# zfountas/deep-active-inference-mc

Hardware: AMD Instinct MI355X
Metric: EFE rollouts/sec (64x64 dSprites, 10 MC-samples, depth 5) (higher is better)
Workload: dtype f32; 1 GPU; calculate_G_repeated: 128 rows (32 roots x 4 actions) x depth 5 x 10 MC samples per GPU (BASELINE configs[1]) + action posterior; rows_per_gpu=128, samples=10, depth=5, parallelism=episodes sharded x1, weights replicated

## Files before the change

deep-active-inference-mc_amd/csrc/decoder.hip:

```cpp
#include <utility>
#include "mfma_pipe.h"

namespace efe {

template <class F, int... I> __device__ __forceinline__ void static_for_(F&& f, std::integer_sequence<int, I...>) { (f(std::integral_constant<int, I>{}), ...); }
template <int N, class F> __device__ __forceinline__ void static_for(F&& f) { static_for_(f, std::make_integer_sequence<int, N>{}); }

__host__ __device__ constexpr int w3_nch(int G) { return G == 4 ? 5 : 4; }
__host__ __device__ constexpr int w3_prod(int G, int c) {
    return G < 4 ? 5 * ((G >> 1) + 2 * (c >> 1)) + (G & 1) + 2 * (c & 1)
         : G == 4 ? (c < 2 ? 5 * (1 + 2 * c) + 4 : c < 4 ? 20 + 1 + 2 * (c - 2) : 24)
                  : (c < 2 ? 5 * (2 * c) + 4 : 20 + 2 * (c - 2));
}
__host__ __device__ constexpr bool w3_direct(int pp) { return f22_o1(pp / 5) < 0 && f22_o1(pp % 5) < 0; }
__host__ __device__ constexpr int w3_view(int pp) { return 3 * f22_view(pp / 5) + f22_view(pp % 5); }
__host__ __device__ constexpr int w3_mat(int pp) { return 4 * f22_wt(pp / 5) + f22_wt(pp % 5); }
__host__ __device__ constexpr bool w3_hits(int pp, int o) {
    const int r = o >> 2, c = o & 3, pr = pp / 5, pc = pp % 5;
    return (r == f22_o0(pr) || r == f22_o1(pr)) && (c == f22_o0(pc) || c == f22_o1(pc));
}
__host__ __device__ constexpr bool w3_seen(int G, int c, int o) {
    for (int g = 0; g < G; ++g)
        for (int k = 0; k < w3_nch(g); ++k) if (w3_hits(w3_prod(g, k), o)) return true;
    if (!w3_direct(w3_prod(G, c)))
// ... 396 lines not shown
                for (int ct = 0; ct < 4; ++ct) {
                    const f32x4 bias4 = smv[DA_BIAS + 16 + 4 * ct + g];
                    f22_l2<FUSED>(acc2, aq, wrsrc(W2 + ct * 256), ct < 3 ? 1 : 0, ln, bias4, smv, nb);
                    if (ct < 3) f22_l2_store(acc2, yr, yoff, ct, true);
                }
                if constexpr (!FUSED) load_next(NPE, 2 * NPH);
                f22_l2_store(acc2, yr, yoff, 3, true);
                if constexpr (FUSED) tail(img, nimg, pf);
            } else {
                load_next(0, 2 * NPH);
            }
        }
        __syncthreads();
        img = nimg; nimg = FUSED ? vpark(nnimg) : nnimg;
    }
}

__global__ void __launch_bounds__(256, 2) k_dec_a(const DecAArgs a) {
    extern __shared__ __attribute__((aligned(16))) float4 sm[];
    dec_a_loop<false>(a, sm, [](int, int, f32x4 (&)[16]) {});
}

constexpr int DAS_IN = 6 * 16;
constexpr int DAS_L1 = 4 * 16;
constexpr int DAS_BIAS = (DAS_IN + 1 + DAS_L1 + 2) * DA_PS;
constexpr size_t DAS_LDS_BYTES = (DAS_BIAS + 32) * sizeof(float4);
__global__ void __launch_bounds__(256, 2) k_dec_a_s(const DecAArgs a) {
    extern __shared__ __attribute__((aligned(16))) float4 sm[];
    float4* sin = sm;
    float4* sl1 = sm + (DAS_IN + 1) * DA_PS;
// ... 68 lines not shown
constexpr size_t DA_LDS_BYTES = (DA_BIAS + 33) * sizeof(float4);
int init_dec_b_kernels();
int init_decoder_kernels() {
    if (hipFuncSetAttribute((const void*)k_dec_a, hipFuncAttributeMaxDynamicSharedMemorySize, DA_LDS_BYTES) != hipSuccess) return 1;
    if (hipFuncSetAttribute((const void*)k_dec_a_s, hipFuncAttributeMaxDynamicSharedMemorySize, DAS_LDS_BYTES) != hipSuccess) return 1;
    return init_dec_b_kernels();
}

void launch_dec_a(const DecAArgs& a, hipStream_t st) {
    if (a.parts == 8) {
        hipLaunchKernelGGL(k_dec_a_s, dim3(a.rows * 8), dim3(256), DAS_LDS_BYTES, st, a);
        return;
    }
    const size_t lds = DA_LDS_BYTES;
    const int grid = a.rows < 512 ? a.rows : 512;
    hipLaunchKernelGGL(k_dec_a, dim3(grid), dim3(256), lds, st, a);
}


template <int PARTS, bool FUSED>
__device__ __forceinline__ void dec_b_image(const DecBArgs& a, float4* const sm, float4* const sb3, float* const sq, float* const sQ,
                                            const int img, const int qtr, const float* const y2img) {
    constexpr int SR = 4, NW = 4, NTHR = 256;
    constexpr int DB_RP = 33;
    constexpr int DB_PS = 17;
    constexpr int DB_IN_F4 = (SR + 1) * DB_RP * DB_PS;
    constexpr int DB_YROWS = 4 * SR + 2;
    constexpr int NPF = (SR + 1) * 512 / NTHR;
    constexpr int NS = 32 / SR;
    float* sH = reinterpret_cast<float*>(sm + DB_IN_F4);
    int tid = threadIdx.x;
// ... 223 lines not shown
        const DecAArgs an = karg_reload<DecAArgs>(kp_lo, kp_hi, 0);
        int tl = threadIdx.x; asm volatile("" : "+v"(tl));
        const int pimg = __builtin_amdgcn_readfirstlane(nimg < an.rows ? nimg : img);
        dec_a_load_x4(pf, an.x4, pimg, __builtin_amdgcn_readfirstlane(tl >> 6), tl, 0, 16);
    }, kp_lo, kp_hi);
}

int init_dec_b_kernels() {
    if (hipFuncSetAttribute((const void*)k_dec_b4<1>, hipFuncAttributeMaxDynamicSharedMemorySize, DB_LDS4D) != hipSuccess) return 1;
    if (hipFuncSetAttribute((const void*)k_dec_b4<4>, hipFuncAttributeMaxDynamicSharedMemorySize, DB_LDS4D) != hipSuccess) return 1;
    return 0;
}

int dec_ab_grid(int rows, int cap) { const int g = rows < 512 ? rows : 512; return cap > 0 && cap < g ? cap : g; }
void launch_dec_ab(const DecABArgs& a, int grid_cap, hipStream_t st) {
    hipLaunchKernelGGL(k_dec_ab, dim3(dec_ab_grid(a.a.rows, grid_cap)), dim3(256), 0, st, a);
}

void launch_dec_b(const DecBArgs& a, hipStream_t st) {
    if (a.parts == 4) hipLaunchKernelGGL(k_dec_b4<4>, dim3(a.rows * 4), dim3(256), DB_LDS4D, st, a);
    else hipLaunchKernelGGL(k_dec_b4<1>, dim3(a.rows), dim3(256), DB_LDS4D, st, a);
}

__host__ __device__ inline int fc4_spg(int mtiles) { return ((mtiles + 7) / 8 + 7) / 8; }
template <int NT>
__global__ void __launch_bounds__(256, 2) k_fc4(const GemmArgs a) {
    constexpr int RT = 32 * NT;
    extern __shared__ __attribute__((aligned(16))) float4 sm[];
    const int tid = threadIdx.x;
    const int lane = tid & 63;
    const int w = __builtin_amdgcn_readfirstlane(tid >> 6);
// ... 93 lines not shown
```

deep-active-inference-mc_amd/csrc/engine.h:

```cpp
#pragma once
#include <hip/hip_runtime.h>
#include <algorithm>
#include <cmath>
#include <cstdio>
#include <cstring>
#include <map>
#include <mutex>
#include <string>
#include <vector>
#include "../../include/efe_engine.h"
#include "ctx_registry.h"
#include "kernels.h"

using namespace efe;

#define HIPCHK(x) do { hipError_t e_ = (x); if (e_ != hipSuccess) { return ctx->fail(std::string(#x) + ": " + hipGetErrorString(e_)); } } while (0)

namespace efe {
namespace host {

constexpr int S_DIM = 10;
constexpr int64_t MAC_TRANS = 541696, MAC_DEC = 43256320, MAC_ENC = 3868960, MAC_HABIT = 18176;
constexpr size_t SCRATCH_HEADROOM = (size_t)1 << 20;

// ... 40 lines not shown
    int pi_dim = 4, chan = 1, res = 64;
    bool generic = false;
    bool last_s1 = false;
    int base = 16, enc_hw[5] = {64, 31, 15, 7, 3};
    size_t img_store = 4096;
    Layer g_fc4, g_ct[3], g_enc[4];
    float* g_wf = nullptr; float g_bf[4] = {0.f, 0.f, 0.f, 0.f};
    float* g_enc1p = nullptr;
    int64_t mac_dec = 43256320, mac_enc = 3868960, mac_trans = 541696, mac_habit = 18176;
    MlpW dec16{}, enc16{};
    int enc16_kc0 = 0;
    int64_t head_unfused = 0;
    MlpW mid16{}, top16{};
    TrainPart top_train, mid_train;
    int64_t mid_unfused = 0;
    float *enc_w1 = nullptr, *enc_b1 = nullptr, *dec_wf = nullptr;
    float dec_bf = 0.f;
    float* dec_raw = nullptr;
    float* dect_raw = nullptr;
    float* dect_raw_g = nullptr;
    float* dec_raw_g = nullptr;
    float* enc_raw = nullptr;
    float* enc_raw_g = nullptr;
    float* down_master = nullptr;
    RepackDesc* down_repack = nullptr; int down_repack_n = 0, down_repack_blocks = 0;
    bool down_dirty = false, dec_bf_stale = false;
    float* down_master_g = nullptr;
    RepackDesc* down_repack_g = nullptr; int down_repack_g_n = 0, down_repack_g_blocks = 0;
    bool g_bf_stale = false;
    float* zeros = nullptr;
// ... 15 lines not shown
    int64_t dec_split = 1;
    int64_t dec_fuse_ab = 1;
    int64_t dec_ab_grid = 0;
    int64_t fuse_final_g = 1;
    int64_t mfma_bf16x3 = 0;
    int split_packed = 0;
    uint16_t* fc4_b3 = nullptr;
    uint16_t* ct_b3[2] = {nullptr, nullptr};
    uint16_t* ct3_b3 = nullptr;
    float s_fc4 = 1.f, s_ct[2] = {1.f, 1.f}, s_ct3 = 1.f;
    int64_t b3_convt3 = 1;
    bool arch_gfx950 = false;
    int64_t sim_split = 1;
    bool sim_sync_dirty = false;
    double* mi_ws = nullptr;
    float* sim_xch = nullptr; int* sim_sync = nullptr;
    int64_t check_rows = 0;
    int64_t last_macs = 0;
    unsigned prof = 0;
    int cls = PROF_OTHER;
    std::vector<hipEvent_t> ev_pool;
    size_t ev_used = 0;
    std::vector<std::pair<int, std::pair<hipEvent_t, hipEvent_t>>> ev_spans;
    hipEvent_t ev_get() {
        if (ev_used == ev_pool.size()) { hipEvent_t e; (void)hipEventCreate(&e); ev_pool.push_back(e); }
        return ev_pool[ev_used++];
    }
    int trace_n = 0;
    hipEvent_t prof_begin(hipStream_t st) {
        if (trace) { (void)hipStreamSynchronize(st); fprintf(stderr, "[efe trace] launch %d class %d ...\n", ++trace_n, cls); fflush(stderr); return (hipEvent_t)1; }
// ... 89 lines not shown
    hipStream_t st;
    bool ok = false, record = false;
    Call(efe_ctx* c, Mode mode, hipStream_t stream = nullptr)
        : adm(registry().admit(c)), ctx(adm.ctx.get()), dev(ctx ? ctx->device : -1), st(stream) { tl_stale_msg.clear(); ok = ctx && !start(mode); }
    int refused(const char* who) const {
        if (!ctx) tl_stale_msg = std::string(who) + ": stale or invalid context handle";
        return 1;
    }
    int start(Mode mode) {
        if (mode == Mode::scratch && !ctx->committed) return ctx->fail("weights not committed");
        if (mode != Mode::host && hipSetDevice(ctx->device) != hipSuccess) return ctx->fail("hipSetDevice failed");
        if (mode == Mode::host || mode == Mode::device) return 0;
        if (ctx->have_last && ctx->last_stream != st && !capturing(st) && hipStreamWaitEvent(st, ctx->done_ev, 0) != hipSuccess)
            return ctx->fail("hipStreamWaitEvent failed");
        ctx->arena.reset();
        if (ctx->poison >= 0)
            for (auto& b : ctx->arena.blocks)
                if (hipMemsetAsync(b.first, (int)(ctx->poison & 0xff), b.second, st) != hipSuccess) return ctx->fail("poison memset failed");
        ctx->last_macs = 0;
        record = true;
        return 0;
    }
    ~Call() {
        if (record && !capturing(st) && hipEventRecord(ctx->done_ev, st) == hipSuccess) { ctx->last_stream = st; ctx->have_last = true; }
        if (ctx) ctx->pending.clear();
    }
    explicit operator bool() const { return ok; }
    int finish() {
        if (!ctx->pending.empty()) return ctx->fail(ctx->pending);
        hipError_t e = hipGetLastError();
        return e == hipSuccess ? 0 : ctx->fail(std::string("kernel launch: ") + hipGetErrorString(e));
    }
};

LayerSpec top_layer(int i, int A);
LayerSpec mid_layer(int i, int A);
int part_param_count(int nl, LayerSpec (*layer)(int, int), int A);
int refresh_down_host(efe_ctx* ctx);
int64_t down_g_count(const efe_ctx* ctx);
int pack_fc4_b3(efe_ctx* ctx, int mode);

NoiseCfg make_noise(uint32_t k0, uint32_t k1, int rows_per_group, uint32_t row_offset, GroupMap gm, const int32_t* ids = nullptr, int div = 1,
                    const uint8_t* mask = nullptr);
NoiseCfg pass_noise(const efe_noise* nz, uint32_t pass, uint32_t sample, int M);
RolloutPlan rollout_plan(const efe_ctx* ctx, int64_t M);
size_t plan_bytes(const efe_ctx* c, const RolloutPlan& p);
DecTailPlan dec_tail_plan(int64_t M, bool own_y1, bool own_y2, bool own_y3, bool own_po);
DecHeadPlan dec_head_plan(int64_t M, bool own_h1, bool own_h2, bool own_h3, bool own_h4);
size_t encoder_bytes(const efe_ctx* ctx, int64_t N);
size_t core_bytes(const efe_ctx* ctx, int64_t R, int64_t D, int64_t S, bool own_terms);
int run_mid(efe_ctx* ctx, const float* X, int x_mod, int M, float* tr , const NoiseCfg& nc, hipStream_t st);
int run_decoder(efe_ctx* ctx, const float* dec_in , int N, const NoiseCfg& nc, int reward0, int store0,
                float* val , float* po_store, hipStream_t st);
int run_encoder(efe_ctx* ctx, const float* o, int N, const NoiseCfg& nc, float* enc, hipStream_t st);
int run_habit(efe_ctx* ctx, const float* s16 , int M, float* l32 , hipStream_t st);
int run_core(efe_ctx* ctx, const CoreIO& io, hipStream_t st);

int fe_params(efe_ctx* ctx, const efe_fe_params* p, bool derived_ok, const char* who);
void fe_omega(FeArgs& a, const efe_fe_params* p);
FeArgs fe_down_args(efe_ctx* ctx, int M, const float* o1, const float* enc, const float* p1_mean, const float* p1_lv, int p1_ld,
                    const efe_fe_params* p, const float* omega, const efe_fe_out* out);

}
}
```

deep-active-inference-mc_amd/csrc/engine_ctx.hip:

```cpp
#include "engine.h"

namespace {

void release_ctx(efe_ctx* ctx) {
    for (hipEvent_t e : ctx->ev_pool) (void)hipEventDestroy(e);
    if (ctx->done_ev) (void)hipEventDestroy(ctx->done_ev);
    for (void* p : ctx->owned) (void)hipFree(p);
    for (void* p : ctx->wbufs) (void)hipFree(p);
    for (auto& b : ctx->arena.blocks) (void)hipFree(b.first);
    delete ctx;
}
void destroy_ctx(efe_ctx* ctx) {
    DeviceScope dev_scope_(ctx->device);
    (void)hipSetDevice(ctx->device);
    (void)hipDeviceSynchronize();
    release_ctx(ctx);
}

}

namespace efe {
namespace host {

bool capturing(hipStream_t st) {
// ... 48 lines not shown
    }
    ctx->mac_trans = (int64_t)(pi_dim + 10) * 512 + 2 * 512 * 512 + 512 * 20;
    ctx->mac_habit = 10 * 128 + 128 * 128 + 128 * pi_dim;
    const size_t zeros_bytes = std::max<size_t>(8192, ((size_t)ctx->enc_hw[4] * ctx->enc_hw[4] * 64 + 64) * sizeof(float));
    if (hipMalloc((void**)&ctx->zeros, zeros_bytes) != hipSuccess) { release_ctx(ctx); return 4; }
    ctx->owned.push_back(ctx->zeros);
    if (hipMemset(ctx->zeros, 0, zeros_bytes) != hipSuccess) { release_ctx(ctx); return 4; }
    if (hipEventCreateWithFlags(&ctx->done_ev, hipEventDisableTiming) != hipSuccess) { ctx->done_ev = nullptr; release_ctx(ctx); return 6; }
    {
        const size_t xb = (size_t)SIM_MAX_SPLIT_GROUPS * 2 * 16 * 512 * sizeof(float), sb = (size_t)SIM_MAX_SPLIT_GROUPS * 4 * sizeof(int);
        if (hipMalloc((void**)&ctx->sim_xch, xb) != hipSuccess) { release_ctx(ctx); return 4; }
        ctx->owned.push_back(ctx->sim_xch);
        if (hipMalloc((void**)&ctx->sim_sync, sb) != hipSuccess) { release_ctx(ctx); return 4; }
        ctx->owned.push_back(ctx->sim_sync);
        if (hipMemset(ctx->sim_sync, 0, sb) != hipSuccess) { release_ctx(ctx); return 4; }
    }
    {
        if (hipMalloc((void**)&ctx->mi_ws, (EVAL_MI_WS + EVAL_MI_PSI) * sizeof(double)) != hipSuccess) { release_ctx(ctx); return 4; }
        ctx->owned.push_back(ctx->mi_ws);
        std::vector<double> psi(EVAL_MI_PSI);
        eval_mi_psi_table(psi.data());
        if (hipMemcpy(ctx->mi_ws + EVAL_MI_WS, psi.data(), psi.size() * sizeof(double), hipMemcpyHostToDevice) != hipSuccess) { release_ctx(ctx); return 4; }
    }
    registry().insert(ctx);
    *out = ctx;
    return 0;
}

void efe_destroy(efe_ctx* ctx) { registry().retire(ctx); }

// ... 45 lines not shown
    if (!strcmp(name, "mfma_bf16x3") || !strcmp(name, "mfma_f16x2")) {
        const int mode = !value ? 0 : name[5] == 'b' ? 1 : 2;
        if (mode && ctx->generic) return ctx->fail(std::string(name) + ": the experiment covers the Dynamic-dSprites geometry only");
        if (mode && ctx->committed && ctx->split_packed != mode) {
            HIPCHK(hipSetDevice(ctx->device));
            HIPCHK(hipDeviceSynchronize());
            if (refresh_down_host(ctx)) return 1;
            if (pack_fc4_b3(ctx, mode)) { ctx->mfma_bf16x3 = 0; return 1; }
        }
        ctx->mfma_bf16x3 = mode;
        return 0;
    }
    if (!strcmp(name, "b3_convt3")) { ctx->b3_convt3 = value ? 1 : 0; return 0; }
    if (!strcmp(name, "arena_align")) { if (value < 256 || (value & (value - 1))) return ctx->fail("arena_align must be a power of two >= 256"); ctx->arena_align = value; return 0; }
    if (!strcmp(name, "mid_unfused")) { ctx->mid_unfused = value; return 0; }
    if (!strcmp(name, "head_unfused")) { ctx->head_unfused = value; return 0; }
    if (!strcmp(name, "enc_chunk")) { if (value < 1) return ctx->fail("enc_chunk < 1"); ctx->enc_chunk = value; return 0; }
    return ctx->fail(std::string("unknown option ") + name);
}

int64_t efe_last_call_macs(efe_ctx* ctx) { Call call(ctx, Mode::host); return call ? ctx->last_macs : 0; }

int efe_prof_enable(efe_ctx* ctx, int on) {
    Call call(ctx, Mode::host); if (!call) return 1;
    ctx->prof = (on < 0) ? 0xFFFFFFFFu : (unsigned)on;
    ctx->ev_used = 0;
    ctx->ev_spans.clear();
    return 0;
}

// ... 49 lines not shown
```

deep-active-inference-mc_amd/csrc/engine_forward.hip:

```cpp
#include "engine.h"

namespace efe {
namespace host {
namespace {

inline RowMask live_of(const NoiseCfg& nc, int m0) { return RowMask{nc.mask, nc.mask_div, m0, nc.rows_per_group, nc.mask ? nc.gm.ids : nullptr}; }
template <class Args>
void set_keys(Args& a, const NoiseCfg& nc, int m0) {
    a.k0 = nc.k0; a.k1 = nc.k1; a.gm = nc.gm; a.rows_per_group = nc.rows_per_group; a.row_offset = nc.row_offset; a.m0 = m0;
}

void fc(efe_ctx* ctx, int cls, const Layer& L, const float* X, int ldx, int x_mod, float* Y, int ldy, int M, bool relu, bool drop,
        uint32_t tag, const NoiseCfg& nc, int m0, hipStream_t st, bool split16 = true) {
    GemmArgs a{};
    a.Wp = L.Wp; a.bias = L.bias; a.X = X; a.Y = Y; a.zeros = ctx->zeros;
    a.n_pix = M; a.cin = L.cin; a.cout = L.cout; a.mtiles = L.mtiles; a.ldx = ldx; a.ldy = ldy; a.x_mod = x_mod;
    a.relu = relu; a.dropout = drop; a.tag = tag;
    set_keys(a, nc, m0);
    ProfSpan span(ctx, cls, st);
    if (L.mtiles >= 64 && !(L.mtiles & 1) && L.cin == 256 && ldx == 256 && x_mod == 0 && relu && drop) {
        if (split16 && ctx->mfma_bf16x3 && ctx->fc4_b3 && &L == &ctx->dec_fc[3]) {
            a.Wb3 = ctx->fc4_b3; a.split = (int)ctx->mfma_bf16x3; a.wb3_scale_inv = 1.0f / ctx->s_fc4;
            launch_fc4_b3(a, st);
        }
// ... 241 lines not shown
    return {(int)C, G, own_y1 ? C * DEC_TAIL_Y1 : 0, own_y2 ? C * DEC_TAIL_Y2 : 0, own_y3 ? C * DEC_TAIL_Y3 : 0, own_po ? C * 4096 : 0,
            C * 4096, C * DEC_TAIL_Y3, C * DEC_TAIL_Y2, C * DEC_TAIL_Y1, G > 1 ? (size_t)G * DEC_TAIL_P : 0};
}
DecHeadPlan dec_head_plan(int64_t M, bool own_h1, bool own_h2, bool own_h3, bool own_h4) {
    const size_t C = (size_t)std::min<int64_t>(DEC_TAIL_ROWS, M);
    const int G = dec_head_slabs((int)std::min<int64_t>(M, 16 * DEC_HEAD_SLABS));
    return {(int)C, G, own_h1 ? C * 256 : 0, own_h2 ? C * 256 : 0, own_h3 ? C * 256 : 0, own_h4 ? C * DEC_TAIL_Y1 : 0, C * DEC_TAIL_Y1,
            (size_t)DEC_HEAD_SEGS * C * 256, G > 1 ? (size_t)G * DEC_HEAD_SMALL_P : 0};
}
size_t encoder_bytes(const efe_ctx* ctx, int64_t N) { return ctx->generic ? plan_bytes(ctx, enc_g_plan(ctx, N)) : plan_bytes(ctx, enc_plan(ctx, N)); }
size_t core_bytes(const efe_ctx* ctx, int64_t R, int64_t D, int64_t S, bool own_terms) {
    return plan_bytes(ctx, core_plan(ctx, R, D, S, true, own_terms)) + (size_t)D * plan_bytes(ctx, mid_plan(ctx, 2 * S * R))
         + decoder_bytes(ctx, D * 3 * S * R) + encoder_bytes(ctx, D * S * R);
}

int run_mid(efe_ctx* ctx, const float* X, int x_mod, int M, float* tr , const NoiseCfg& nc, hipStream_t st) {
    ctx->last_macs += (int64_t)M * ctx->mac_trans;
    if (!ctx->mid_unfused) {
        TransFusedArgs a{};
        a.W = ctx->mid16; a.X = X; a.tr = tr; a.M = M; a.x_mod = x_mod;
        set_keys(a, nc, 0);
        ProfSpan span(ctx, PROF_MID, st);
        launch_trans_fused(a, st);
        return 0;
    }
    const MidPlan p = mid_plan(ctx, M);
    float* h1 = ctx->allocT<float>(p.h1);
    float* h2 = ctx->allocT<float>(p.h2);
    if (!h1 || !h2) return 1;
    fc(ctx, PROF_MID, ctx->mid[0], X, 16, x_mod, h1, 512, M, true, true, TAG_MID + 0, nc, 0, st);
    fc(ctx, PROF_MID, ctx->mid[1], h1, 512, 0, h2, 512, M, true, true, TAG_MID + 1, nc, 0, st);
    fc(ctx, PROF_MID, ctx->mid[2], h2, 512, 0, h1, 512, M, true, true, TAG_MID + 2, nc, 0, st);
    fc(ctx, PROF_MID, ctx->mid[3], h1, 512, 0, tr, 32, M, false, false, 0, nc, 0, st);
    return 0;
}

// ... 10 lines not shown
    }
    const DecPlan p = dec_plan(ctx, N);
    const bool split = p.split;
    const bool f16 = ctx->mfma_bf16x3 == 2;
    const bool fc4_16 = !(f16 && split), ct3_16 = ctx->b3_convt3 || f16;
    const int C = p.C;
    float* hA = ctx->allocT<float>(p.hA);
    float* hB = ctx->allocT<float>(p.hB);
    float* x4 = ctx->allocT<float>(p.x4);
    float* y2 = ctx->allocT<float>(p.y2);
    if (!hA || !hB || !x4 || !y2) return 1;
    ctx->last_macs += (int64_t)N * ctx->mac_dec;
    dense_head(ctx, false, dec_in, 16, hA, 256, hA, hB, N, nc, 0, st);
    int* queues = ctx->allocT<int>(p.queues);
    if (!queues) return 1;
    if (!split && hipMemsetAsync(queues, 0, p.queues * sizeof(int), st) != hipSuccess) return ctx->fail("hipMemsetAsync failed");
    for (int m0 = 0; m0 < N; m0 += C) {
        const int c = std::min(C, N - m0);
        fc(ctx, PROF_DEC_FC4, ctx->dec_fc[3], hA + (size_t)m0 * 256, 256, 0, x4, 16384, c, true, true, TAG_DEC + 3, nc, m0, st, fc4_16);
        if (p.fused) {
            DecABArgs ab{};
            DecAArgs& da = ab.a; DecBArgs& db = ab.b;
            da.x4 = x4; da.y2 = y2; da.w1 = ctx->dec_ct[0].Wp; da.b1 = ctx->dec_ct[0].bias; da.w2 = ctx->dec_ct[1].Wp;
            da.b2 = ctx->dec_ct[1].bias; da.rows = c; da.live = live_of(nc, m0); da.queue = queues + m0 / C; da.parts = 1;
            db.y2 = y2; db.w3 = ctx->dec_ct[2].Wp; db.b3 = ctx->dec_ct[2].bias; db.w4 = ctx->dec_wf; db.b4 = ctx->dec_bf;
            db.rows = c; db.live = da.live; db.m0 = m0; db.rows_per_group = nc.rows_per_group; db.gm = nc.gm; db.reward0 = reward0; db.store0 = store0;
            db.val = val; db.parts = 1; db.valq = nullptr; db.po = po_store; db.reward_intent = (int)ctx->reward_intent;
            ProfSpan span(ctx, PROF_CT2, st);
            launch_dec_ab(ab, (int)ctx->dec_ab_grid, st);
            continue;
        }
        DecAArgs da{};
        da.x4 = x4; da.y2 = y2; da.w1 = ctx->dec_ct[0].Wp; da.b1 = ctx->dec_ct[0].bias; da.w2 = ctx->dec_ct[1].Wp;
        da.b2 = ctx->dec_ct[1].bias; da.rows = c; da.live = live_of(nc, m0); da.queue = queues + m0 / C; da.parts = split ? 8 : 1;
        {
            ProfSpan span(ctx, PROF_CT2, st);
            if (ctx->mfma_bf16x3 && ctx->ct_b3[0] && !split) {
                da.w1b3 = ctx->ct_b3[0]; da.w2b3 = ctx->ct_b3[1]; da.split = (int)ctx->mfma_bf16x3;
                da.w1s = ctx->s_ct[0]; da.w1s_inv = 1.0f / ctx->s_ct[0]; da.w2s = ctx->s_ct[1]; da.w2s_inv = 1.0f / ctx->s_ct[1];
                launch_dec_a_b3(da, st);
            }
            else launch_dec_a(da, st);
        }
        DecBArgs db{};
        db.y2 = y2; db.w3 = ctx->dec_ct[2].Wp; db.b3 = ctx->dec_ct[2].bias; db.w4 = ctx->dec_wf; db.b4 = ctx->dec_bf;
        db.rows = c; db.live = live_of(nc, m0); db.m0 = m0; db.rows_per_group = nc.rows_per_group; db.gm = nc.gm; db.reward0 = reward0; db.store0 = store0;
        db.val = val; db.parts = split ? 4 : 1; db.valq = split ? val : nullptr; db.po = po_store; db.reward_intent = (int)ctx->reward_intent;
        ProfSpan span(ctx, PROF_CT3, st);
        if (ctx->mfma_bf16x3 && ct3_16 && ctx->ct3_b3 && !split) {
// ... 49 lines not shown
    float* xbuf = ctx->allocT<float>(plan.xbuf);
    float* val = ctx->allocT<float>(plan.val);
    float* po_store = ctx->allocT<float>(plan.po_store);
    float* enc = ctx->allocT<float>(plan.enc);
    float* terms_tmp = io.terms ? nullptr : ctx->allocT<float>(plan.terms_tmp);
    if (!tr_all || !dec_in || !xbuf || !val || !po_store || !enc) return 1;
    auto noise = [&](const GroupMap& gm, const uint8_t* mask) { return make_noise(io.k0, io.k1, R, io.row_offset, gm, io.ids, io.mask_div, mask); };

    const float* x = io.x0;
    for (int t = 0; t < D; ++t) {
        float* tr = tr_all + (size_t)t * 2 * S * R * 32;
        if (io.pre_tr) {
        } else if (io.given_mean) {
            launch_fill_tr(io.given_mean, io.given_logvar, tr, R, st);
            if (run_mid(ctx, x, R, R, tr + (size_t)R * 32, noise(GroupMap{1, 1, {PASS_T2, 0, 0}, io.stage0 + (uint32_t)t, 0}, nullptr), st)) return 1;
        } else {
            if (run_mid(ctx, x, R, 2 * S * R, tr, noise(GroupMap{2 * S, S, {PASS_T1, PASS_T2, 0}, io.stage0 + (uint32_t)t, 0}, nullptr), st)) return 1;
        }
        TransPostArgs p{};
        p.tr = tr; p.x = x; p.eps_inj = io.eps ? io.eps + (size_t)t * 3 * S * R * 10 : nullptr;
        p.given_ps1 = io.given_ps1;
        p.dec_in = dec_in + (size_t)t * 3 * S * R * 16;
        float* nx = xbuf + (size_t)(t & 1) * R * 16;
        p.next_x = (t + 1 < D) ? nx : nullptr;
        p.ps1_last = (t + 1 == D) ? io.ps1 : nullptr;
        p.ps1_mean_last = (t + 1 == D) ? io.ps1_mean : nullptr;
        p.S = S; p.R = R; p.mean_mode = io.mean_mode; p.carry_mean = io.carry_mean;
        p.k0 = io.k0; p.k1 = io.k1; p.stage = io.stage0 + t; p.row_offset = io.row_offset; p.pi_dim = ctx->pi_dim;
        p.ids = io.ids; p.ids_div = io.mask_div;
        launch_trans_post(p, st);
        x = nx;
    }
    if (run_decoder(ctx, dec_in, D * 3 * S * R, noise(GroupMap{3 * S, S, {PASS_D1, PASS_D2A, PASS_D2B}, io.stage0, 0}, io.mask), 1, 1, val, po_store, st)) return 1;
    if (run_encoder(ctx, po_store, D * S * R, noise(GroupMap{S, S, {PASS_E1, 0, 0}, io.stage0, 0}, io.mask), enc, st)) return 1;
    TermsArgs ta{};
    ta.val = val; ta.valq = plan.vsplit ? val : nullptr; ta.tr = tr_all; ta.enc = enc; ta.D = D; ta.S = S; ta.R = R;
    ta.reward_div = ctx->generic ? 0.0f : (ctx->reward_intent ? 192.0f : 4096.0f);
    ta.G = io.G; ta.terms = io.terms ? io.terms : terms_tmp; ta.t2parts = io.t2parts;
    launch_terms(ta, st);
    if (io.po1) {
        const float* last = po_store + ((size_t)(D - 1) * S + (S - 1)) * R * ctx->img_store;
        if (ctx->generic) launch_to_nchw(last, io.po1, R, ctx->res * ctx->res, ctx->chan, st);
        else if (hipMemcpyAsync(io.po1, last, (size_t)R * 4096 * 4, hipMemcpyDeviceToDevice, st) != hipSuccess) return ctx->fail("po1 copy failed");
    }
    return 0;
// ... 5 lines not shown
```

deep-active-inference-mc_amd/csrc/fused.hip:

```cpp
#include "kernels.h"

namespace efe {

typedef float f32x4 __attribute__((ext_vector_type(4)));
typedef unsigned u32x4 __attribute__((ext_vector_type(4)));

namespace {

constexpr int FR = 16;
constexpr int ACT_F4 = FR * 128;

__device__ __forceinline__ int aswz(int n, int c4) { return n * 128 + ((c4 & ~15) | ((c4 ^ n) & 15)); }

__device__ __forceinline__ float4 wfrag16(__amdgpu_buffer_rsrc_t r, unsigned lane_bytes, unsigned f4_index) {
    const u32x4 v = __builtin_amdgcn_raw_buffer_load_b128(r, lane_bytes, f4_index * 16u, 0);
    return __builtin_bit_cast(float4, v);
}
__device__ __forceinline__ __amdgpu_buffer_rsrc_t rsrc16(const void* base) {
    return __builtin_amdgcn_make_buffer_rsrc(const_cast<void*>(base), 0, 0x7fffffff, 0x00020000);
}

#define MFMA16(ACC, AV, BV)                                                     \
    ACC = __builtin_amdgcn_mfma_f32_16x16x4f32((AV).x, (BV).x, ACC, 0, 0, 0);   \
    ACC = __builtin_amdgcn_mfma_f32_16x16x4f32((AV).y, (BV).y, ACC, 0, 0, 0);   \
// ... 154 lines not shown
        const float4 v = hidden16_slice<true, true>(W.w[1], W.b[1], mt0, 32, bufB, n, q, ln, k0, k1, TAG_MID + 1, rk);
        float* xb = xch + (size_t)(xn & 1) * (16 * 512);
        __builtin_amdgcn_raw_buffer_store_b128(__builtin_bit_cast(u32x4, v), rsrc16(xb), (unsigned)((n * XCH_ROW_F4 + 4 * mt0 + q) * 16), 0, AUX_SC1);
        xchg_gather<NWG>(xb, sync, NWG * (xn + 1), bufA, tid, bad);
        ++xn;
    }
    {
        const float4 v = hidden16_slice<true, true>(W.w[2], W.b[2], mt0, 32, bufA, n, q, ln, k0, k1, TAG_MID + 2, rk);
        float* xb = xch + (size_t)(xn & 1) * (16 * 512);
        __builtin_amdgcn_raw_buffer_store_b128(__builtin_bit_cast(u32x4, v), rsrc16(xb), (unsigned)((n * XCH_ROW_F4 + 4 * mt0 + q) * 16), 0, AUX_SC1);
        xchg_gather<NWG>(xb, sync, NWG * (xn + 1), bufB, tid, bad);
        ++xn;
    }
    if (w < 2) bufA[aswz(n, 4 * w + q)] = hidden16_slice<false, false>(W.w[3], W.b[3], w, 32, bufB, n, q, ln, k0, k1, 0u, rk);
    __syncthreads();
}

}

__global__ void __launch_bounds__(256, 2) k_trans_fused(const TransFusedArgs a) {
    extern __shared__ __attribute__((aligned(16))) float4 sm[];
    float4* bufA = sm;
    float4* bufB = sm + ACT_F4;
    const int tid = threadIdx.x, lane = tid & 63;
    const int w = __builtin_amdgcn_readfirstlane(tid >> 6);
    const int n = lane & 15, q = lane >> 4;
    const unsigned ln = (unsigned)lane * 16u;
    const int row0 = blockIdx.x * FR;
    {
        if (tid < 64) {
// ... 12 lines not shown
        const int mg = a.m0 + m;
        const int g = mg / a.rows_per_group;
        rk.row = global_row(a.gm.ids, a.gm.ids_div, mg - g * a.rows_per_group, a.row_offset);
        const uint2 key = group_key(a.gm, g);
        rk.stream = key.x; rk.stage = key.y;
    }
    __syncthreads();
    trans_chain(a.W, bufA, bufB, w, n, q, ln, a.k0, a.k1, rk);
    if (tid < 64) {
        const int m = row0 + n;
        if (m < a.M) {
            reinterpret_cast<float4*>(a.tr + (size_t)m * 32)[q] = bufA[aswz(n, q)];
            reinterpret_cast<float4*>(a.tr + (size_t)m * 32)[4 + q] = bufA[aswz(n, 4 + q)];
        }
    }
}

void launch_trans_fused(const TransFusedArgs& a, hipStream_t st) {
    hipLaunchKernelGGL(k_trans_fused, dim3((a.M + FR - 1) / FR), dim3(256), 2 * ACT_F4 * sizeof(float4), st, a);
}

template <int NWG>
__global__ void __launch_bounds__(256, 1) k_sim_chain(const SimChainArgs a) {
    extern __shared__ __attribute__((aligned(16))) float4 sm[];
    float4* bufA = sm;
    float4* bufB = sm + ACT_F4;
    float* srow = reinterpret_cast<float*>(sm + 2 * ACT_F4);
    float* sact = srow + SIM_FE * 16;
    const int A = a.pi_dim;
    const int tid = threadIdx.x, lane = tid & 63;
// ... 266 lines not shown
```

deep-active-inference-mc_amd/csrc/kernels.h:

```cpp
#pragma once
#include <hip/hip_runtime.h>
#include <stdint.h>
#include "philox.h"

namespace efe {

struct GroupMap {
    int per_stage, S;
    uint32_t pass[3];
    uint32_t stage0, sample0;
    const int32_t* ids = nullptr; int ids_div = 1;
};
__device__ __forceinline__ uint32_t global_row(const int32_t* ids, int ids_div, int r, uint32_t row_offset) {
    if (!ids) return row_offset + (uint32_t)r;
    const int e = r / ids_div;
    return row_offset + (uint32_t)(ids[e] * ids_div + (r - e * ids_div));
}
__host__ __device__ inline void group_decode(const GroupMap& gm, int g, int& t, int& pidx, int& samp) {
    t = g / gm.per_stage;
    const int q = g - t * gm.per_stage;
    pidx = q / gm.S;
    samp = q - pidx * gm.S;
}
__device__ __forceinline__ uint2 group_key(const GroupMap& gm, int g) {
// ... 50 lines not shown
    uint32_t row_offset;
    int m0;
    const void* Wb3 = nullptr;
    int split = 0;
    float wb3_scale_inv = 1.0f;
};

struct DecAArgs {
    const float* x4; float* y2;
    const float* w1; const float* b1;
    const float* w2; const float* b2;
    int rows;
    RowMask live;
    int parts;
    int* queue;
    const void* w1b3 = nullptr; const void* w2b3 = nullptr;
    int split = 0;
    float w1s = 1.0f, w1s_inv = 1.0f, w2s = 1.0f, w2s_inv = 1.0f;
};
__host__ __device__ constexpr int f22_view(int p) { return p == 4 ? 2 : (p & 1); }
__host__ __device__ constexpr int f22_wt(int p) { return p < 2 ? 0 : p - 1; }
__host__ __device__ constexpr int f22_o0(int p) { return p < 2 ? 0 : (p < 4 ? 1 : 3); }
__host__ __device__ constexpr int f22_o1(int p) { return p == 1 ? 2 : (p == 3 ? 3 : -1); }
__host__ __device__ constexpr int f22_cw(int wt, int k) { return wt == 0 ? (k == 1) : wt == 1 ? (k == 2) : wt == 2 ? (k != 1) : (k == 0); }
__host__ __device__ inline float f22_u_elem(const float* k, int wr, int wc) {
#pragma clang fp contract(off)
    double s = 0;
    for (int kh = 0; kh < 3; ++kh)
        for (int kw = 0; kw < 3; ++kw) s += (double)(f22_cw(wr, kh) * f22_cw(wc, kw)) * (double)k[kh * 3 + kw];
    return (float)s;
}
__host__ __device__ constexpr double wino_g(int a, int u) { return a == 0 ? (u == 0 ? 1.0 : 0.0) : a == 1 ? 0.5 : a == 2 ? (u == 1 ? -0.5 : 0.5) : (u == 2 ? 1.0 : 0.0); }
__host__ __device__ inline float wino_u_elem(const float* k, int a, int b) {
#pragma clang fp contract(off)
    double Gg[3];
    for (int v = 0; v < 3; ++v) {
        double s = 0;
        for (int u = 0; u < 3; ++u) s += wino_g(a, u) * (double)k[(2 - u) * 3 + (2 - v)];
        Gg[v] = s;
    }
    double s = 0;
    for (int v = 0; v < 3; ++v) s += Gg[v] * wino_g(b, v);
    return (float)s;
}

struct DecBArgs {
    const float* y2;
    const float* w3; const float* b3;
    const float* w4; float b4;
    int rows;
    RowMask live;
    int m0;
    int rows_per_group;
    GroupMap gm;
    int reward0;
    int store0;
    float* val;
    int parts;
    float* valq;
    float* po;
// ... 93 lines not shown

struct MlpW { const float4* w[4]; const float* b[4]; };
struct HeadArgs {
    MlpW W;
    int kc0;
    int nl;
    int out_tiles;
    uint32_t tag0;
    const float* X; float* Y;
    int M;
    uint32_t k0, k1;
    GroupMap gm; int rows_per_group; uint32_t row_offset; int m0;
};
void launch_head(const HeadArgs& a, hipStream_t st);

struct TransFusedArgs {
    MlpW W;
    const float* X;
    float* tr;
    int M, x_mod;
    uint32_t k0, k1;
    GroupMap gm; int rows_per_group; uint32_t row_offset; int m0;
};
void launch_trans_fused(const TransFusedArgs& a, hipStream_t st);
struct SimChainArgs {
    MlpW W, H;
    const float* s0;
    int E, T, use_means;
    uint32_t k0, k1, stage, row_offset;
    const float* eps_inj;
    const float* u_inj;
    float *s0_traj, *ps1_traj, *mean_traj, *lv_traj;
    float* pi0;
    float* Qpi0;
    float* tr;
    int pi_dim;
    const int32_t* ids;
// ... 500 lines not shown
```

Before: 12700 rollouts/s.

## Fold trans-post into fused transition kernel and self-reset decoder work queue

Adds a fold path that performs the trans_post sampling (reparameterized noise, dec_in/next_x writes) inside the fused transition MLP kernel, removing a separate launch per depth step. It also gives the decoder a persistent queue counter that the last ticket-holding block resets to zero, so the per-call hipMemsetAsync can be skipped. fold_trans_post defaults to off while fold_launches defaults to on, so only the queue self-reset is active by default. The risk is queue state desync if a launch aborts, plus duplicated noise logic in the fold path.

```diff
diff --git a/deep-active-inference-mc_amd/csrc/decoder.hip b/deep-active-inference-mc_amd/csrc/decoder.hip
--- a/deep-active-inference-mc_amd/csrc/decoder.hip
+++ b/deep-active-inference-mc_amd/csrc/decoder.hip
@@ -434,6 +434,12 @@
         __syncthreads();
         img = nimg; nimg = FUSED ? vpark(nnimg) : nnimg;
     }
+    int te_ = tid; asm volatile("" : "+v"(te_));
+    if (te_ == 0) {
+        int* const queue = FUSED ? karg_reload<int*>(kp_lo, kp_hi, __builtin_offsetof(DecAArgs, queue)) : a_.queue;
+        const int last = FUSED ? karg_reload<int>(kp_lo, kp_hi, __builtin_offsetof(DecAArgs, last_ticket)) : a_.last_ticket;
+        if (slot[0] == last) *queue = 0;
+    }
 }
 
 __global__ void __launch_bounds__(256, 2) k_dec_a(const DecAArgs a) {
@@ -532,7 +538,9 @@
     }
     const size_t lds = DA_LDS_BYTES;
     const int grid = a.rows < 512 ? a.rows : 512;
-    hipLaunchKernelGGL(k_dec_a, dim3(grid), dim3(256), lds, st, a);
+    DecAArgs al = a;
+    al.last_ticket = dec_last_ticket(grid, a.rows);
+    hipLaunchKernelGGL(k_dec_a, dim3(grid), dim3(256), lds, st, al);
 }
 
 
@@ -786,7 +794,10 @@
 
 int dec_ab_grid(int rows, int cap) { const int g = rows < 512 ? rows : 512; return cap > 0 && cap < g ? cap : g; }
 void launch_dec_ab(const DecABArgs& a, int grid_cap, hipStream_t st) {
-    hipLaunchKernelGGL(k_dec_ab, dim3(dec_ab_grid(a.a.rows, grid_cap)), dim3(256), 0, st, a);
+    const int grid = dec_ab_grid(a.a.rows, grid_cap);
+    DecABArgs al = a;
+    al.a.last_ticket = dec_last_ticket(grid, a.a.rows);
+    hipLaunchKernelGGL(k_dec_ab, dim3(grid), dim3(256), 0, st, al);
 }
 
 void launch_dec_b(const DecBArgs& a, hipStream_t st) {
diff --git a/deep-active-inference-mc_amd/csrc/engine.h b/deep-active-inference-mc_amd/csrc/engine.h
--- a/deep-active-inference-mc_amd/csrc/engine.h
+++ b/deep-active-inference-mc_amd/csrc/engine.h
@@ -78,6 +78,8 @@
     MlpW mid16{}, top16{};
     TrainPart top_train, mid_train;
     int64_t mid_unfused = 0;
+    int64_t fold_launches = 1;
+    int64_t fold_trans_post = 0;
     float *enc_w1 = nullptr, *enc_b1 = nullptr, *dec_wf = nullptr;
     float dec_bf = 0.f;
     float* dec_raw = nullptr;
@@ -123,6 +125,7 @@
     int64_t sim_split = 1;
     bool sim_sync_dirty = false;
     double* mi_ws = nullptr;
+    int* dec_queue = nullptr; int dec_queue_state = 0;
     float* sim_xch = nullptr; int* sim_sync = nullptr;
     int64_t check_rows = 0;
     int64_t last_macs = 0;
@@ -242,6 +245,7 @@
         if (ctx->have_last && ctx->last_stream != st && !capturing(st) && hipStreamWaitEvent(st, ctx->done_ev, 0) != hipSuccess)
             return ctx->fail("hipStreamWaitEvent failed");
         ctx->arena.reset();
+        if (ctx->dec_queue_state == 2) ctx->dec_queue_state = 1;
         if (ctx->poison >= 0)
             for (auto& b : ctx->arena.blocks)
                 if (hipMemsetAsync(b.first, (int)(ctx->poison & 0xff), b.second, st) != hipSuccess) return ctx->fail("poison memset failed");
@@ -257,6 +261,7 @@
     int finish() {
         if (!ctx->pending.empty()) return ctx->fail(ctx->pending);
         hipError_t e = hipGetLastError();
+        if (e == hipSuccess && ctx->dec_queue_state == 2) ctx->dec_queue_state = 0;
         return e == hipSuccess ? 0 : ctx->fail(std::string("kernel launch: ") + hipGetErrorString(e));
     }
 };
@@ -277,7 +282,7 @@
 DecHeadPlan dec_head_plan(int64_t M, bool own_h1, bool own_h2, bool own_h3, bool own_h4);
 size_t encoder_bytes(const efe_ctx* ctx, int64_t N);
 size_t core_bytes(const efe_ctx* ctx, int64_t R, int64_t D, int64_t S, bool own_terms);
-int run_mid(efe_ctx* ctx, const float* X, int x_mod, int M, float* tr , const NoiseCfg& nc, hipStream_t st);
+int run_mid(efe_ctx* ctx, const float* X, int x_mod, int M, float* tr , const NoiseCfg& nc, hipStream_t st, const TransFoldArgs* fold = nullptr);
 int run_decoder(efe_ctx* ctx, const float* dec_in , int N, const NoiseCfg& nc, int reward0, int store0,
                 float* val , float* po_store, hipStream_t st);
 int run_encoder(efe_ctx* ctx, const float* o, int N, const NoiseCfg& nc, float* enc, hipStream_t st);
diff --git a/deep-active-inference-mc_amd/csrc/engine_ctx.hip b/deep-active-inference-mc_amd/csrc/engine_ctx.hip
--- a/deep-active-inference-mc_amd/csrc/engine_ctx.hip
+++ b/deep-active-inference-mc_amd/csrc/engine_ctx.hip
@@ -86,6 +86,11 @@
         if (hipMalloc((void**)&ctx->sim_sync, sb) != hipSuccess) { release_ctx(ctx); return 4; }
         ctx->owned.push_back(ctx->sim_sync);
         if (hipMemset(ctx->sim_sync, 0, sb) != hipSuccess) { release_ctx(ctx); return 4; }
+    }
+    {
+        if (hipMalloc((void**)&ctx->dec_queue, 256) != hipSuccess) { release_ctx(ctx); return 4; }
+        ctx->owned.push_back(ctx->dec_queue);
+        if (hipMemset(ctx->dec_queue, 0, 256) != hipSuccess) { release_ctx(ctx); return 4; }
     }
     {
         if (hipMalloc((void**)&ctx->mi_ws, (EVAL_MI_WS + EVAL_MI_PSI) * sizeof(double)) != hipSuccess) { release_ctx(ctx); return 4; }
@@ -161,6 +166,8 @@
     if (!strcmp(name, "b3_convt3")) { ctx->b3_convt3 = value ? 1 : 0; return 0; }
     if (!strcmp(name, "arena_align")) { if (value < 256 || (value & (value - 1))) return ctx->fail("arena_align must be a power of two >= 256"); ctx->arena_align = value; return 0; }
     if (!strcmp(name, "mid_unfused")) { ctx->mid_unfused = value; return 0; }
+    if (!strcmp(name, "fold_launches")) { ctx->fold_launches = value ? 1 : 0; return 0; }
+    if (!strcmp(name, "fold_trans_post")) { ctx->fold_trans_post = value ? 1 : 0; return 0; }
     if (!strcmp(name, "head_unfused")) { ctx->head_unfused = value; return 0; }
     if (!strcmp(name, "enc_chunk")) { if (value < 1) return ctx->fail("enc_chunk < 1"); ctx->enc_chunk = value; return 0; }
     return ctx->fail(std::string("unknown option ") + name);
diff --git a/deep-active-inference-mc_amd/csrc/engine_forward.hip b/deep-active-inference-mc_amd/csrc/engine_forward.hip
--- a/deep-active-inference-mc_amd/csrc/engine_forward.hip
+++ b/deep-active-inference-mc_amd/csrc/engine_forward.hip
@@ -279,12 +279,13 @@
          + decoder_bytes(ctx, D * 3 * S * R) + encoder_bytes(ctx, D * S * R);
 }
 
-int run_mid(efe_ctx* ctx, const float* X, int x_mod, int M, float* tr , const NoiseCfg& nc, hipStream_t st) {
+int run_mid(efe_ctx* ctx, const float* X, int x_mod, int M, float* tr , const NoiseCfg& nc, hipStream_t st, const TransFoldArgs* fold) {
     ctx->last_macs += (int64_t)M * ctx->mac_trans;
     if (!ctx->mid_unfused) {
         TransFusedArgs a{};
         a.W = ctx->mid16; a.X = X; a.tr = tr; a.M = M; a.x_mod = x_mod;
         set_keys(a, nc, 0);
+        if (fold) a.fold = *fold;
         ProfSpan span(ctx, PROF_MID, st);
         launch_trans_fused(a, st);
         return 0;
@@ -325,7 +326,11 @@
     dense_head(ctx, false, dec_in, 16, hA, 256, hA, hB, N, nc, 0, st);
     int* queues = ctx->allocT<int>(p.queues);
     if (!queues) return 1;
-    if (!split && hipMemsetAsync(queues, 0, p.queues * sizeof(int), st) != hipSuccess) return ctx->fail("hipMemsetAsync failed");
+    const bool own_queue = ctx->fold_launches && !split;
+    if (own_queue) {
+        if (ctx->dec_queue_state == 1 && hipMemsetAsync(ctx->dec_queue, 0, sizeof(int), st) != hipSuccess) return ctx->fail("hipMemsetAsync failed");
+        ctx->dec_queue_state = 2;
+    } else if (!split && hipMemsetAsync(queues, 0, p.queues * sizeof(int), st) != hipSuccess) return ctx->fail("hipMemsetAsync failed");
     for (int m0 = 0; m0 < N; m0 += C) {
         const int c = std::min(C, N - m0);
         fc(ctx, PROF_DEC_FC4, ctx->dec_fc[3], hA + (size_t)m0 * 256, 256, 0, x4, 16384, c, true, true, TAG_DEC + 3, nc, m0, st, fc4_16);
@@ -333,7 +338,7 @@
             DecABArgs ab{};
             DecAArgs& da = ab.a; DecBArgs& db = ab.b;
             da.x4 = x4; da.y2 = y2; da.w1 = ctx->dec_ct[0].Wp; da.b1 = ctx->dec_ct[0].bias; da.w2 = ctx->dec_ct[1].Wp;
-            da.b2 = ctx->dec_ct[1].bias; da.rows = c; da.live = live_of(nc, m0); da.queue = queues + m0 / C; da.parts = 1;
+            da.b2 = ctx->dec_ct[1].bias; da.rows = c; da.live = live_of(nc, m0); da.queue = own_queue ? ctx->dec_queue : queues + m0 / C; da.parts = 1;
             db.y2 = y2; db.w3 = ctx->dec_ct[2].Wp; db.b3 = ctx->dec_ct[2].bias; db.w4 = ctx->dec_wf; db.b4 = ctx->dec_bf;
             db.rows = c; db.live = da.live; db.m0 = m0; db.rows_per_group = nc.rows_per_group; db.gm = nc.gm; db.reward0 = reward0; db.store0 = store0;
             db.val = val; db.parts = 1; db.valq = nullptr; db.po = po_store; db.reward_intent = (int)ctx->reward_intent;
@@ -343,7 +348,7 @@
         }
         DecAArgs da{};
         da.x4 = x4; da.y2 = y2; da.w1 = ctx->dec_ct[0].Wp; da.b1 = ctx->dec_ct[0].bias; da.w2 = ctx->dec_ct[1].Wp;
-        da.b2 = ctx->dec_ct[1].bias; da.rows = c; da.live = live_of(nc, m0); da.queue = queues + m0 / C; da.parts = split ? 8 : 1;
+        da.b2 = ctx->dec_ct[1].bias; da.rows = c; da.live = live_of(nc, m0); da.queue = own_queue ? ctx->dec_queue : queues + m0 / C; da.parts = split ? 8 : 1;
         {
             ProfSpan span(ctx, PROF_CT2, st);
             if (ctx->mfma_bf16x3 && ctx->ct_b3[0] && !split) {
@@ -423,8 +428,6 @@
         } else if (io.given_mean) {
             launch_fill_tr(io.given_mean, io.given_logvar, tr, R, st);
             if (run_mid(ctx, x, R, R, tr + (size_t)R * 32, noise(GroupMap{1, 1, {PASS_T2, 0, 0}, io.stage0 + (uint32_t)t, 0}, nullptr), st)) return 1;
-        } else {
-            if (run_mid(ctx, x, R, 2 * S * R, tr, noise(GroupMap{2 * S, S, {PASS_T1, PASS_T2, 0}, io.stage0 + (uint32_t)t, 0}, nullptr), st)) return 1;
         }
         TransPostArgs p{};
         p.tr = tr; p.x = x; p.eps_inj = io.eps ? io.eps + (size_t)t * 3 * S * R * 10 : nullptr;
@@ -437,7 +440,12 @@
         p.S = S; p.R = R; p.mean_mode = io.mean_mode; p.carry_mean = io.carry_mean;
         p.k0 = io.k0; p.k1 = io.k1; p.stage = io.stage0 + t; p.row_offset = io.row_offset; p.pi_dim = ctx->pi_dim;
         p.ids = io.ids; p.ids_div = io.mask_div;
-        launch_trans_post(p, st);
+        if (!io.pre_tr && !io.given_mean) {
+            const bool fold = ctx->fold_trans_post && !ctx->mid_unfused;
+            const TransFoldArgs f{p.eps_inj, p.given_ps1, p.dec_in, p.next_x, p.ps1_last, p.ps1_mean_last, p.mean_mode, p.carry_mean, p.pi_dim};
+            if (run_mid(ctx, x, R, 2 * S * R, tr, noise(GroupMap{2 * S, S, {PASS_T1, PASS_T2, 0}, io.stage0 + (uint32_t)t, 0}, nullptr), st, fold ? &f : nullptr)) return 1;
+            if (!fold) launch_trans_post(p, st);
+        } else launch_trans_post(p, st);
         x = nx;
     }
     if (run_decoder(ctx, dec_in, D * 3 * S * R, noise(GroupMap{3 * S, S, {PASS_D1, PASS_D2A, PASS_D2B}, io.stage0, 0}, io.mask), 1, 1, val, po_store, st)) return 1;
diff --git a/deep-active-inference-mc_amd/csrc/fused.hip b/deep-active-inference-mc_amd/csrc/fused.hip
--- a/deep-active-inference-mc_amd/csrc/fused.hip
+++ b/deep-active-inference-mc_amd/csrc/fused.hip
@@ -192,6 +192,72 @@
     }
     if (w < 2) bufA[aswz(n, 4 * w + q)] = hidden16_slice<false, false>(W.w[3], W.b[3], w, 32, bufB, n, q, ln, k0, k1, 0u, rk);
     __syncthreads();
+}
+
+__device__ __forceinline__ void normal_quad(float (&z)[4], uint32_t k0, uint32_t k1, uint32_t row, uint32_t stream, uint32_t stage, uint32_t blk) {
+    const uint4 w = noise_words(k0, k1, TAG_EPS, blk, row, stream, stage);
+    const float r0 = sqrtf(-2.0f * logf(u01(w.x))), th0 = 6.283185307179586f * u01(w.y);
+    const float r1 = sqrtf(-2.0f * logf(u01(w.z))), th1 = 6.283185307179586f * u01(w.w);
+    z[0] = r0 * cosf(th0); z[1] = r0 * sinf(th0); z[2] = r1 * cosf(th1); z[3] = r1 * sinf(th1);
+}
+
+__device__ __forceinline__ void trans_fold(const TransFusedArgs& a, const float* out, const int row0, const int tid) {
+    const TransFoldArgs& p = a.fold;
+    const int S = a.gm.S, R = a.rows_per_group;
+    const int blk = tid & 3, nn = (tid >> 2) & 15;
+    const int m = row0 + nn;
+    if (m >= a.M) return;
+    const int g = m / R, r = m - g * R;
+    const bool last1 = g == S - 1;
+    const int T = (row0 < S * R && row0 + FR > (S - 1) * R) ? 1 + S : 1;
+    float mean[4], sd[4];
+#pragma unroll
+    for (int e = 0; e < 4; ++e) {
+        const int k = 4 * blk + e;
+        mean[e] = 0.f; sd[e] = 0.f;
+        if (k < 10) {
+            mean[e] = out[aswz(nn, k >> 2) * 4 + (k & 3)];
+            sd[e] = expf(out[aswz(nn, (10 + k) >> 2) * 4 + ((10 + k) & 3)] * 0.5f);
+        }
+    }
+    const uint32_t grow = global_row(a.gm.ids, a.gm.ids_div, r, a.row_offset);
+    for (int t = tid >> 6; t < T; t += 4) {
+        if (t > 0 && !last1) continue;
+        const int qd = t == 0 ? g : 2 * S + t - 1;
+        const uint32_t pass = t > 0 ? PASS_D2B : (g < S ? PASS_T1 : PASS_T2);
+        const uint32_t sample = (uint32_t)(t > 0 ? t - 1 : (g < S ? g : g - S));
+        const bool use_mean = t == 0 && p.mean_mode;
+        const size_t dr = (size_t)qd * R + r;
+        float z[4] = {0.f, 0.f, 0.f, 0.f};
+        if (blk < 3) {
+            if (p.eps_inj) {
+#pragma unroll
+                for (int e = 0; e < 4; ++e)
+                    if (4 * blk + e < 10) z[e] = p.eps_inj[dr * 10 + 4 * blk + e];
+            } else normal_quad(z, a.k0, a.k1, grow, stream_id(pass, sample), a.gm.stage0, (uint32_t)blk);
+        }
+        float o[4];
+#pragma unroll
+        for (int e = 0; e < 4; ++e) {
+            const int k = 4 * blk + e;
+            o[e] = 0.f;
+            if (k < 10) {
+                const float samp = z[e] * sd[e] + mean[e];
+                o[e] = use_mean ? mean[e] : samp;
+                if (t == 0 && last1) {
+                    if (p.ps1_last) p.ps1_last[(size_t)r * 10 + k] = samp;
+                    if (p.ps1_mean_last) p.ps1_mean_last[(size_t)r * 10 + k] = mean[e];
+                    if (p.next_x) p.next_x[(size_t)r * 16 + p.pi_dim + k] = (p.carry_mean || p.mean_mode) ? mean[e] : samp;
+                    if (p.given_ps1) o[e] = p.given_ps1[(size_t)r * 10 + k];
+                }
+            }
+            if (t == 0 && last1 && p.next_x) {
+                if (k < p.pi_dim) p.next_x[(size_t)r * 16 + k] = a.X[(size_t)r * 16 + k];
+                if (k >= p.pi_dim + 10) p.next_x[(size_t)r * 16 + k] = 0.0f;
+            }
+        }
+        reinterpret_cast<float4*>(p.dec_in + dr * 16)[blk] = make_float4(o[0], o[1], o[2], o[3]);
+    }
 }
 
 }
@@ -234,6 +300,7 @@
             reinterpret_cast<float4*>(a.tr + (size_t)m * 32)[4 + q] = bufA[aswz(n, 4 + q)];
         }
     }
+    if (a.fold.dec_in) trans_fold(a, reinterpret_cast<const float*>(bufA), row0, tid);
 }
 
 void launch_trans_fused(const TransFusedArgs& a, hipStream_t st) {
diff --git a/deep-active-inference-mc_amd/csrc/kernels.h b/deep-active-inference-mc_amd/csrc/kernels.h
--- a/deep-active-inference-mc_amd/csrc/kernels.h
+++ b/deep-active-inference-mc_amd/csrc/kernels.h
@@ -88,6 +88,7 @@
     RowMask live;
     int parts;
     int* queue;
+    int last_ticket;
     const void* w1b3 = nullptr; const void* w2b3 = nullptr;
     int split = 0;
     float w1s = 1.0f, w1s_inv = 1.0f, w2s = 1.0f, w2s_inv = 1.0f;
@@ -118,6 +119,7 @@
     return (float)s;
 }
 
+inline int dec_last_ticket(int grid, int rows) { return 2 * grid + (grid < rows ? grid : rows) + rows - 1; }
 struct DecBArgs {
     const float* y2;
     const float* w3; const float* b3;
@@ -241,6 +243,11 @@
 };
 void launch_head(const HeadArgs& a, hipStream_t st);
 
+struct TransFoldArgs {
+    const float* eps_inj; const float* given_ps1;
+    float* dec_in; float* next_x; float* ps1_last; float* ps1_mean_last;
+    int mean_mode, carry_mean, pi_dim;
+};
 struct TransFusedArgs {
     MlpW W;
     const float* X;
@@ -248,6 +255,7 @@
     int M, x_mod;
     uint32_t k0, k1;
     GroupMap gm; int rows_per_group; uint32_t row_offset; int m0;
+    TransFoldArgs fold;
 };
 void launch_trans_fused(const TransFusedArgs& a, hipStream_t st);
 struct SimChainArgs {
```

Measured after the change: 12710 rollouts/s (median of 2 runs). Within noise of the previous version (+0.1%).
